# locuslab/mpc.pytorch

Measured on NVIDIA H100. Metric: LQR solves/sec, higher is better.
Workload: dtype f32

## Files before the change

### include/mpcb200.h

```cpp
#ifndef MPCB200_H_
#define MPCB200_H_

#include <stddef.h>
#include <stdint.h>

#ifdef __cplusplus
extern "C" {
#endif

#define MPCB200_VERSION 2

enum {
  MPCB200_OK = 0,
  MPCB200_ERR_NULL_POINTER = 1,
  MPCB200_ERR_BAD_DIMS = 2,
  MPCB200_ERR_UNSUPPORTED_DIMS = 3,
  MPCB200_ERR_SMEM = 4,
  MPCB200_ERR_LAUNCH = 5,
  MPCB200_ERR_NO_DEVICE = 6,
  MPCB200_ERR_NO_GRAPH_COND = 7
};

typedef struct mpcb200_dims {
  int32_t B;
// ... 105 lines not shown
} mpcb200_ilqr_opts;

size_t mpcb200_ilqr_workspace_bytes(const mpcb200_dims* dims, const mpcb200_ilqr_opts* opts, int32_t elem_size);
int mpcb200_ilqr_f32(const mpcb200_dims* dims, const mpcb200_params* params, const mpcb200_ilqr_opts* opts,
                     const float* C, const float* c, const float* F, const float* f,
                     const float* x_init, const float* u_init,
                     const float* u_lower, const float* u_upper, const uint8_t* u_zero_I,
                     float* best_x, float* best_u, float* best_costs, float* best_full_du_norm,
                     int32_t* info, void* workspace, size_t workspace_bytes, void* stream);
int mpcb200_ilqr_f64(const mpcb200_dims* dims, const mpcb200_params* params, const mpcb200_ilqr_opts* opts,
                     const double* C, const double* c, const double* F, const double* f,
                     const double* x_init, const double* u_init,
                     const double* u_lower, const double* u_upper, const uint8_t* u_zero_I,
                     double* best_x, double* best_u, double* best_costs, double* best_full_du_norm,
                     int32_t* info, void* workspace, size_t workspace_bytes, void* stream);

int mpcb200_supported(int32_t n_state, int32_t n_ctrl);

int mpcb200_supported_list(int32_t* out, int32_t cap);

uint64_t mpcb200_launch_count(void);

size_t mpcb200_step_smem_bytes(const mpcb200_dims* dims, int32_t elem_size);

int mpcb200_step_prefers_workspace(const mpcb200_dims* dims, int32_t elem_size);

#define MPCB200_PLAN_GENERIC 1u
#define MPCB200_PLAN_PAIR 2u
#define MPCB200_PLAN_GAINS_SMEM 4u
#define MPCB200_PLAN_KREDUCE 8u
#define MPCB200_PLAN_LARGE 16u
int32_t mpcb200_last_step_plan(void);

int mpcb200_version(void);
const char* mpcb200_strerror(int code);

#ifdef __cplusplus
}
#endif
#endif
```

### mpc/pytorch_b200/_lib.py

```python
import contextlib
import ctypes
import functools
import os

import torch

_HERE = os.path.dirname(os.path.abspath(__file__))
LIB_PATH = os.environ.get("MPCB200_LIB", os.path.join(_HERE, "libmpcb200.so"))


class Dims(ctypes.Structure):
    _fields_ = [(k, ctypes.c_int32) for k in (
        "B", "T", "n", "m", "F_T", "has_f", "bounds_kind", "has_zero_mask",
        "has_delta_u", "max_ls_iter", "pnqp_max_iter", "do_rollout", "dynamics_kind", "reserved0")] + \
        [(k, ctypes.c_int64) for k in ("C_tstride", "c_tstride", "F_tstride", "f_tstride")]



class Params(ctypes.Structure):
    _fields_ = [(k, ctypes.c_double) for k in ("u_lo", "u_hi", "delta_u", "ls_decay")] + [("dyn", ctypes.c_double * 8)]


class IlqrOpts(ctypes.Structure):
    _fields_ = [(k, ctypes.c_int32) for k in ("lqr_iter", "not_improved_lim", "m_ref", "reserved0")] + \
        [(k, ctypes.c_double) for k in ("eps", "best_cost_eps")]


class MpcB200Error(RuntimeError):
    pass


ERR_NO_GRAPH_COND = 7


_lib = None

EXPORTED_SYMBOLS = (
    "mpcb200_lqr_step_f32", "mpcb200_lqr_step_f64", "mpcb200_lqr_grad_f32", "mpcb200_lqr_grad_f64",
    "mpcb200_rollout_f32", "mpcb200_rollout_f64", "mpcb200_pnqp_f32", "mpcb200_pnqp_f64", "mpcb200_pnqp_max_n",
    "mpcb200_lqr_adjoint_f32", "mpcb200_lqr_adjoint_f64", "mpcb200_adjoint_workspace_bytes",
    "mpcb200_dyn_rollout_f32", "mpcb200_dyn_rollout_f64", "mpcb200_dyn_linearize_f32", "mpcb200_dyn_linearize_f64",
    "mpcb200_supported", "mpcb200_supported_list", "mpcb200_launch_count",
    "mpcb200_step_smem_bytes", "mpcb200_step_prefers_workspace", "mpcb200_last_step_plan", "mpcb200_version",
    "mpcb200_strerror", "mpcb200_step_large_fits", "mpcb200_ilqr_f32", "mpcb200_ilqr_f64",
    "mpcb200_ilqr_workspace_bytes",
)

PLAN_GENERIC, PLAN_PAIR, PLAN_GAINS_SMEM, PLAN_KREDUCE, PLAN_LARGE = 1, 2, 4, 8, 16


def lib():
    global _lib
    if _lib is not None:
        return _lib
    if not os.path.exists(LIB_PATH):
        raise MpcB200Error(
            f"{LIB_PATH} is not built. Run `python -c 'import __graft_entry__ as g; g.build()'` "
            "(or `make -C mpc/pytorch_b200/csrc`). There is no CPU fallback.")
    L = ctypes.CDLL(LIB_PATH)
    vp = ctypes.c_void_p
    step_args = [ctypes.POINTER(Dims), ctypes.POINTER(Params)] + [vp] * 22
    for name in ("mpcb200_lqr_step_f32", "mpcb200_lqr_step_f64"):
        fn = getattr(L, name)
        fn.argtypes = step_args
        fn.restype = ctypes.c_int
    grad_args = [ctypes.POINTER(Dims)] + [vp] * 15
    for name in ("mpcb200_lqr_grad_f32", "mpcb200_lqr_grad_f64"):
        fn = getattr(L, name)
        fn.argtypes = grad_args
        fn.restype = ctypes.c_int
    for name in ("mpcb200_rollout_f32", "mpcb200_rollout_f64"):
        fn = getattr(L, name)
        fn.argtypes = [ctypes.POINTER(Dims)] + [vp] * 6
        fn.restype = ctypes.c_int
    for name in ("mpcb200_pnqp_f32", "mpcb200_pnqp_f64"):
        fn = getattr(L, name)
        fn.argtypes = [ctypes.c_int32, ctypes.c_int32] + [vp] * 5 + [ctypes.c_int32] + [vp] * 6
        fn.restype = ctypes.c_int
# ... 4 lines not shown
        fn.argtypes = [ctypes.POINTER(Dims), ctypes.POINTER(Params)] + [vp] * 15 + [ctypes.c_size_t, vp]
        fn.restype = ctypes.c_int
    L.mpcb200_adjoint_workspace_bytes.argtypes = [ctypes.POINTER(Dims), ctypes.c_int32]
    L.mpcb200_adjoint_workspace_bytes.restype = ctypes.c_size_t
    for name in ("mpcb200_dyn_rollout_f32", "mpcb200_dyn_rollout_f64"):
        fn = getattr(L, name)
        fn.argtypes = [ctypes.c_int32, ctypes.POINTER(ctypes.c_double), ctypes.c_int32, ctypes.c_int32] + [vp] * 4
        fn.restype = ctypes.c_int
    for name in ("mpcb200_dyn_linearize_f32", "mpcb200_dyn_linearize_f64"):
        fn = getattr(L, name)
        fn.argtypes = [ctypes.c_int32, ctypes.POINTER(ctypes.c_double), ctypes.c_int32, ctypes.c_int32] + [vp] * 5
        fn.restype = ctypes.c_int
    for name in ("mpcb200_ilqr_f32", "mpcb200_ilqr_f64"):
        fn = getattr(L, name)
        fn.argtypes = [ctypes.POINTER(Dims), ctypes.POINTER(Params), ctypes.POINTER(IlqrOpts)] + [vp] * 15 + \
            [ctypes.c_size_t, vp]
        fn.restype = ctypes.c_int
    L.mpcb200_ilqr_workspace_bytes.argtypes = [ctypes.POINTER(Dims), ctypes.POINTER(IlqrOpts), ctypes.c_int32]
    L.mpcb200_ilqr_workspace_bytes.restype = ctypes.c_size_t
    L.mpcb200_supported.argtypes = [ctypes.c_int32, ctypes.c_int32]
    L.mpcb200_supported.restype = ctypes.c_int
    L.mpcb200_supported_list.argtypes = [ctypes.POINTER(ctypes.c_int32), ctypes.c_int32]
    L.mpcb200_supported_list.restype = ctypes.c_int
    L.mpcb200_launch_count.argtypes = []
    L.mpcb200_launch_count.restype = ctypes.c_uint64
    L.mpcb200_step_smem_bytes.argtypes = [ctypes.POINTER(Dims), ctypes.c_int32]
    L.mpcb200_step_smem_bytes.restype = ctypes.c_size_t
    L.mpcb200_step_prefers_workspace.argtypes = [ctypes.POINTER(Dims), ctypes.c_int32]
    L.mpcb200_step_prefers_workspace.restype = ctypes.c_int
    L.mpcb200_step_large_fits.argtypes = [ctypes.POINTER(Dims), ctypes.c_int32]
    L.mpcb200_step_large_fits.restype = ctypes.c_int
    L.mpcb200_last_step_plan.argtypes = []
    L.mpcb200_last_step_plan.restype = ctypes.c_int32
    L.mpcb200_version.argtypes = []
    L.mpcb200_version.restype = ctypes.c_int
    L.mpcb200_strerror.argtypes = [ctypes.c_int]
    L.mpcb200_strerror.restype = ctypes.c_char_p
    _lib = L
    return L


_DTYPE_SUFFIX = {torch.float32: "_f32", torch.float64: "_f64"}


@functools.cache
def entry(name, dtype):
    suffix = _DTYPE_SUFFIX.get(dtype)
    if suffix is None:
        raise MpcB200Error(f"unsupported dtype {dtype}")
    return getattr(lib(), name + suffix)


def check(rc, what):
    if rc != 0:
        raise MpcB200Error(f"{what} failed: [{rc}] {lib().mpcb200_strerror(rc).decode()}")


def supported_pairs():
    L = lib()
    n = L.mpcb200_supported_list(None, 0)
    buf = (ctypes.c_int32 * (2 * n))()
    L.mpcb200_supported_list(buf, n)
    return [(buf[2 * i], buf[2 * i + 1]) for i in range(n)]


def launch_count():
    return int(lib().mpcb200_launch_count())


def last_step_plan():
    return int(lib().mpcb200_last_step_plan())


def ptr(t):
    if t is None:
        return None
    if not t.is_cuda:
        raise MpcB200Error("mpc.pytorch_b200 runs on CUDA tensors only (no CPU fallback)")
    if not t.is_contiguous():
        raise MpcB200Error("internal error: non-contiguous tensor reached the C ABI")
    return ctypes.c_void_p(t.data_ptr())


def ptr_view(t):
    if t is None:
        return None
    if not t.is_cuda:
        raise MpcB200Error("mpc.pytorch_b200 runs on CUDA tensors only (no CPU fallback)")
    return ctypes.c_void_p(t.data_ptr())


def stream_handle(device):
    return ctypes.c_void_p(torch.cuda.current_stream(device).cuda_stream)


def _on_device(dev):
    if dev.index is None or dev.index == torch.cuda.current_device():
        return contextlib.nullcontext()
    return torch.cuda.device(dev)
```

### mpc/pytorch_b200/csrc/api.cu

```cuda
#include <atomic>
#include <cstdlib>
#include <cstring>

#include "../../../include/mpcb200.h"
#include "ilqr.cuh"
#include "lqr_grad.cuh"
#include "lqr_large.cuh"
#include "lqr_rollout.cuh"
#include "lqr_step.cuh"
#include "pnqp.cuh"

namespace mpcb200 {
#define MPCB200_INST(n, m)                                                  \
  int step_f32__##n##_##m(const StepArgs&, int, cudaStream_t);              \
  int step_f64__##n##_##m(const StepArgs&, int, cudaStream_t);              \
  int grad_f32__##n##_##m(const GradArgs&, cudaStream_t);                   \
  int grad_f64__##n##_##m(const GradArgs&, cudaStream_t);                   \
  int pws_f32__##n##_##m(int, int);                                         \
  int pws_f64__##n##_##m(int, int);                                         \
  int roll_f32__##n##_##m(const RolloutArgs&, cudaStream_t);                \
  int roll_f64__##n##_##m(const RolloutArgs&, cudaStream_t);                \
  size_t smem_f32__##n##_##m(int);                                          \
  size_t smem_f64__##n##_##m(int);
#include "instances.def"
// ... 7 lines not shown
  int (*grad64)(const GradArgs&, cudaStream_t);
  size_t (*smem32)(int);
  size_t (*smem64)(int);
  int (*roll32)(const RolloutArgs&, cudaStream_t);
  int (*roll64)(const RolloutArgs&, cudaStream_t);
  int (*pws32)(int, int);
  int (*pws64)(int, int);
};
static const Entry kTable[] = {
#define MPCB200_INST(n, m)                                                                  \
  {n, m, step_f32__##n##_##m, step_f64__##n##_##m, grad_f32__##n##_##m, grad_f64__##n##_##m, \
   smem_f32__##n##_##m, smem_f64__##n##_##m, roll_f32__##n##_##m, roll_f64__##n##_##m,   \
   pws_f32__##n##_##m, pws_f64__##n##_##m},
#include "instances.def"
#undef MPCB200_INST
};
static const int kTableLen = (int)(sizeof(kTable) / sizeof(kTable[0]));

static const Entry* find(int n, int m) {
  for (int i = 0; i < kTableLen; ++i)
    if (kTable[i].n == n && kTable[i].m == m) return &kTable[i];
  return nullptr;
}

static bool large_forced() {
  const char* k = std::getenv("MPCB200_KERNEL");
  return k != nullptr && std::atoi(k) == 3;
}
static bool runs_large(int n, int m) { return find(n, m) == nullptr || large_forced(); }
static constexpr int kOptinAssumed = 227 * 1024;

static std::atomic<uint64_t> g_launches{0};
static thread_local int t_step_plan = 0;

void record_step_plan(int plan) { t_step_plan = plan; }

int max_smem_optin() {
  static std::atomic<int> cache[64];
  int dev = 0;
  if (cudaGetDevice(&dev) != cudaSuccess) return -1;
  if (dev < 0 || dev >= 64) return -1;
  if (cache[dev].load(std::memory_order_acquire) == 0) {
    int v = 0, major = 0;
    if (cudaDeviceGetAttribute(&v, cudaDevAttrMaxSharedMemoryPerBlockOptin, dev) != cudaSuccess) return -1;
    if (cudaDeviceGetAttribute(&major, cudaDevAttrComputeCapabilityMajor, dev) != cudaSuccess) return -1;
    if (major != 9) return -1;
    cache[dev].store(v, std::memory_order_release);
  }
  return cache[dev].load(std::memory_order_acquire);
}

struct TimeStrides { long long C, c, F, f; };
static TimeStrides time_strides(const mpcb200_dims* d) {
  auto ts = [](long long given, long long dense) { return given == 0 ? dense : (given < 0 ? 0 : given); };
  const long long B = d->B, n = d->n, p = d->n + d->m;
  return {ts(d->C_tstride, B * p * p), ts(d->c_tstride, B * p), ts(d->F_tstride, B * n * p), ts(d->f_tstride, B * n)};
}

static bool aligned16(const void* p) { return (reinterpret_cast<uintptr_t>(p) & 15u) == 0; }

static int check_dims(const mpcb200_dims* d) {
  if (d == nullptr) return MPCB200_ERR_NULL_POINTER;
  if (d->B <= 0 || d->T <= 0 || d->n <= 0 || d->m <= 0) return MPCB200_ERR_BAD_DIMS;
  if (d->F_T != d->T - 1 && d->F_T != d->T) return MPCB200_ERR_BAD_DIMS;
  return MPCB200_OK;
}

static int check_bounds(const mpcb200_dims* d, const void* lo, const void* hi) {
// ... 67 lines not shown
  const size_t sz = sizeof(R);
  bool ok = aligned16(C) && aligned16(c) && aligned16(cur_x) && aligned16(cur_u) &&
            (F == nullptr || aligned16(F)) && (!d->has_f || aligned16(f)) &&
            (d->bounds_kind != 2 || (aligned16(u_lower) && aligned16(u_upper)));
  ok = ok && (x_init == nullptr || aligned16(x_init));
  ok = ok && ((size_t)d->B * d->m * sz) % 16 == 0 && ((size_t)d->B * d->n * sz) % 16 == 0;
  a.bulk_ok = ok ? 1 : 0;
  const TimeStrides ts = time_strides(d);
  a.C_ts = ts.C; a.c_ts = ts.c; a.F_ts = ts.F; a.f_ts = ts.f;
  ok = ok && (a.C_ts * sz) % 16 == 0 && (a.c_ts * sz) % 16 == 0 && (a.F_ts * sz) % 16 == 0 && (a.f_ts * sz) % 16 == 0;
  a.bulk_ok = ok ? 1 : 0;
  a.dyn_kind = d->dynamics_kind;
  if (a.dyn_kind != DYN_LINEAR) {
    if (!known_shape_ok(d)) return MPCB200_ERR_BAD_DIMS;
    for (int i = 0; i < 8; ++i) a.dp.p[i] = p->dyn[i];
  }
  if (large) {
    if (adj != nullptr) return MPCB200_ERR_UNSUPPORTED_DIMS;
    if (Ks == nullptr) return MPCB200_ERR_SMEM;
    const int n = d->n, m = d->m, p = n + m;
    auto spans = [&](const void* base, long long ts, long long span) {
      return base != nullptr && aligned16(base) && (ts * (long long)sz) % 16 == 0 && (span * (long long)sz) % 16 == 0;
    };
    unsigned bulk = 0u;
    if (spans(C, a.C_ts, (long long)p * p)) bulk |= LB_C;
    if (spans(F, a.F_ts, (long long)n * p)) bulk |= LB_F;
    if (spans(c, a.c_ts, p)) bulk |= LB_c;
    if (d->has_f && spans(f, a.f_ts, n)) bulk |= LB_f;
    if (spans(cur_x, (long long)d->B * n, n)) bulk |= LB_x;
    if (spans(cur_u, (long long)d->B * m, m)) bulk |= LB_u;
    if (d->bounds_kind == 2 && spans(u_lower, (long long)d->B * m, m) && spans(u_upper, (long long)d->B * m, m))
      bulk |= LB_BOX;
    t_step_plan = 0;
    rc = large_step_launch<R>(a, n, m, bulk, smem, (cudaStream_t)stream);
    if (rc == 0) g_launches.fetch_add(1);
    return rc;
  }
  if (const char* k = std::getenv("MPCB200_KERNEL")) a.impl = std::atoi(k);
  if (adj != nullptr) {
    if (!adj->ok || !a.bulk_ok || a.impl == 1) return MPCB200_ERR_UNSUPPORTED_DIMS;
    a.impl = 2;
    a.adj = 1; a.adj_has_df = adj->has_df; a.adj_c = adj->c; a.adj_x = adj->x; a.adj_u = adj->u;
    a.adj_dC = adj->dC; a.adj_dc = adj->dc; a.adj_dF = adj->dF; a.adj_df = adj->df; a.adj_dx_init = adj->dx_init;
    a.adj_c_ts = adj->c_ts;
  }
  t_step_plan = 0;
  rc =(sizeof(R) == 4 ? e->step32 : e->step64)(a, smem, (cudaStream_t)stream);
  if (rc == 0) g_launches.fetch_add(1);
  return rc;
}

template <typename R>
static int grad_impl(const mpcb200_dims* d, const R* C, const R* c, const R* F, const R* new_x,
                     const R* new_u, const R* dx, const R* du, const R* dl_dx, R* dx_init, R* dC, R* dc,
                     R* dF, R* df, void* workspace, void* stream) {
  int rc = check_dims(d);
  if (rc) return rc;
  if (C == nullptr || c == nullptr || new_x == nullptr || new_u == nullptr || dx == nullptr ||
      du == nullptr || dl_dx == nullptr || dx_init == nullptr || dC == nullptr || dc == nullptr)
    return MPCB200_ERR_NULL_POINTER;
  if (d->F_T > 0 && (F == nullptr || dF == nullptr)) return MPCB200_ERR_NULL_POINTER;
  const Entry* e = find(d->n, d->m);
  const bool large = runs_large(d->n, d->m);
  if (max_smem_optin() <= 0) return MPCB200_ERR_NO_DEVICE;
  GradArgs a;
  std::memset(&a, 0, sizeof(a));
  a.B = d->B; a.T = d->T; a.F_T = d->F_T; a.has_df = df != nullptr;
  a.C = C; a.c = c; a.F = F; a.new_x = new_x; a.new_u = new_u; a.dx = dx; a.du = du; a.dl_dx = dl_dx;
  a.dx_init = dx_init; a.dC = dC; a.dc = dc; a.dF = dF; a.df = df; a.workspace = workspace;
  const TimeStrides ts = time_strides(d);
  a.C_ts = ts.C; a.c_ts = ts.c; a.F_ts = ts.F;
  rc = large ? large_grad_launch<R>(a, d->n, d->m, (cudaStream_t)stream)
             : (sizeof(R) == 4 ? e->grad32 : e->grad64)(a, (cudaStream_t)stream);
  if (rc == 0) g_launches.fetch_add(workspace != nullptr ? 2 : 1);
  return rc;
}
struct AdjLayout {
  size_t negr, zeros, dx, du, costate, scal, mask, maskf, Ks, ks, total;
  bool gains;
// ... 482 lines not shown
int mpcb200_supported_list(int32_t* out, int32_t cap) {
  for (int i = 0; i < kTableLen && i < cap; ++i) {
    out[2 * i] = kTable[i].n;
    out[2 * i + 1] = kTable[i].m;
  }
  return kTableLen;
}

uint64_t mpcb200_launch_count(void) { return g_launches.load(); }

size_t mpcb200_step_smem_bytes(const mpcb200_dims* dims, int32_t elem_size) {
  if (dims == nullptr) return 0;
  const Entry* e = find(dims->n, dims->m);
  if (e == nullptr) return 0;
  return elem_size == 8 ? e->smem64(dims->T) : e->smem32(dims->T);
}

int mpcb200_step_prefers_workspace(const mpcb200_dims* dims, int32_t elem_size) {
  if (dims == nullptr) return 0;
  if (runs_large(dims->n, dims->m)) return 1;
  const Entry* e = find(dims->n, dims->m);
  int ms = max_smem_optin();
  if (ms <= 0) ms = kOptinAssumed;
  return elem_size == 8 ? e->pws64(dims->T, ms) : e->pws32(dims->T, ms);
}

int mpcb200_step_large_fits(const mpcb200_dims* dims, int32_t elem_size) {
  if (dims == nullptr || (elem_size != 4 && elem_size != 8)) return 0;
  return large_step_fits(dims->n, dims->m, elem_size, kOptinAssumed) ? 1 : 0;
}

int32_t mpcb200_last_step_plan(void) { return t_step_plan; }

int mpcb200_version(void) { return MPCB200_VERSION; }

const char* mpcb200_strerror(int code) {
  switch (code) {
    case MPCB200_OK: return "ok";
    case MPCB200_ERR_NULL_POINTER: return "a required pointer is NULL";
    case MPCB200_ERR_BAD_DIMS: return "bad dimensions or option combination";
    case MPCB200_ERR_UNSUPPORTED_DIMS: return "no kernel instance compiled for this (n_state, n_ctrl)";
    case MPCB200_ERR_SMEM: return "problem does not fit shared memory (pass Ks/ks buffers for long horizons)";
    case MPCB200_ERR_LAUNCH: return "CUDA launch failed";
    case MPCB200_ERR_NO_DEVICE: return "no usable sm_90 device";
    case MPCB200_ERR_NO_GRAPH_COND: return "conditional CUDA graph nodes are unavailable (driver older than 12.3)";
    default: return "unknown error";
  }
}
}
```

### mpc/pytorch_b200/csrc/lqr_step.cuh

```cuda
#pragma once
#include "../../../include/mpcb200.h"
#include "common.cuh"
#include "dynamics.cuh"

namespace mpcb200 {

struct StepArgs {
  int B, T, F_T;
  int has_f, bounds_kind, has_mask, has_delta, max_ls, pnqp_iters, do_rollout;
  double u_lo, u_hi, delta_u, ls_decay;
  const void *C, *c, *F, *f, *x_init, *cur_x, *cur_u, *u_lower, *u_upper;
  const unsigned char* zero_mask;
  void *new_x, *new_u, *costs, *full_du_norm, *alphas, *du_first;
  int* qp_iters;
  unsigned char* free_mask;
  int* status;
  void *Ks, *ks;
  int bulk_ok;
  int k_in_smem;
  int impl;
  long long C_ts, c_ts, F_ts, f_ts;
  int adj, adj_has_df;
  const void *adj_c, *adj_x, *adj_u;
  void *adj_dC, *adj_dc, *adj_dF, *adj_df, *adj_dx_init;
  long long adj_c_ts;
  int dyn_kind;
  DynParams dp;
};

void record_step_plan(int plan);

template <typename R, int N, int M>
struct StepCfg {
  static constexpr int P = N + M;
  static constexpr int EA = 16 / (int)sizeof(R);
  static_assert(P <= 32, "one problem must fit a warp");
  static constexpr bool STATE_LANES = N == 8 && M == 2 && sizeof(R) == 4;
  static constexpr int LP = STATE_LANES ? N : P;
  static constexpr int CPL = (P + LP - 1) / LP;
  static constexpr int PPW = 32 / LP;
  static constexpr bool x_slot(int sl) { return sl * LP < N; }
  static constexpr bool span_ok(int nw) {
    return (nw * PPW * M * (int)sizeof(R)) % 16 == 0 && (nw * PPW * N * (int)sizeof(R)) % 16 == 0;
  }
  static constexpr int NW = STATE_LANES ? 2 : span_ok(1) ? 1 : span_ok(2) ? 2 : 4;
  static constexpr int W = NW * PPW;
  static_assert(span_ok(NW), "CTA problem count must keep spans 16-byte aligned");
  static constexpr int THREADS = (NW + 1) * 32;
  static constexpr int MIN_CTAS = STATE_LANES ? 32 / W : 0;
  static constexpr int S = 3;
  static constexpr int VS = round_up(N, 4);
  static constexpr int CS = P * P, FS = N * P;
  static constexpr int OFF_C = 0;
  static constexpr int OFF_F = OFF_C + W * CS;
  static constexpr int OFF_c = OFF_F + W * FS;
  static constexpr int OFF_f = OFF_c + W * P;
  static constexpr int OFF_x = OFF_f + W * N;
  static constexpr int OFF_u = OFF_x + W * N;
  static constexpr int OFF_lo = OFF_u + W * M;
  static constexpr int OFF_hi = OFF_lo + W * M;
  static constexpr int OFF_END = OFF_hi + W * M;
  static constexpr int STAGE_BYTES = round_up(OFF_END * (int)sizeof(R) + round_up(W * M, 16), 128);
  static constexpr int SC_V = 0;
  static constexpr int SC_v = SC_V + N * VS;
  static constexpr int SC_K = SC_v + VS;
  static constexpr int KT = M * VS + round_up(M, 4);
  static constexpr int SC_Q = SC_K + KT;
  static constexpr int SC_R = SC_Q + M * VS;
  static constexpr int SC_RAW = SC_R + round_up(P, 4);
  static constexpr int SCR = (SC_RAW % 32 == 0 || SC_RAW % 32 == 16) ? SC_RAW + 4 : SC_RAW;
  static constexpr bool KREDUCE = CPL == 1 && PPW == 1 && (N & (N - 1)) == 0;
  static constexpr int GAIN_SMEM_LIMIT = 6144;
  static bool prefers_workspace(int T, int max_smem_optin) {
    return smem_bytes(T, true) > (size_t)max_smem_optin ||
           (KREDUCE && (size_t)T * KT * sizeof(R) > (size_t)GAIN_SMEM_LIMIT);
  }
  static constexpr int HDR_BYTES = 256;
  static size_t smem_bytes(int T, bool k_in_smem) {
    size_t b = HDR_BYTES + (size_t)S * STAGE_BYTES + (size_t)W * SCR * sizeof(R);
    if (k_in_smem) b += (size_t)W * T * KT * sizeof(R);
    return b;
  }
};

template <typename R, int M>
MPCB_DEV void pnqp_lane(const R (&H)[M][M], const R (&q)[M], const R (&lo)[M], const R (&hi)[M],
                        bool warm, R (&x)[M], Ldl<R, M>& fac, unsigned& fmask, int& iters,
                        bool& conv, bool& badpiv, int max_iter) {
  const R GAMMA = R(0.1);
  auto obj = [&](const R(&z)[M]) {
    R s = R(0);
#pragma unroll
    for (int a = 0; a < M; ++a) {
      R hz = R(0);
#pragma unroll
      for (int b = 0; b < M; ++b) hz += H[a][b] * z[b];
      s += z[a] * (R(0.5) * hz + q[a]);
    }
    return s;
  };
  badpiv = false;
  if (!warm) {
    fac.factor(H);
    badpiv = fac.bad;
    R t[M];
    fac.solve(q, t);
#pragma unroll
    for (int a = 0; a < M; ++a) x[a] = -t[a];
  }
#pragma unroll
  for (int a = 0; a < M; ++a) {
    x[a] = x[a] < lo[a] ? lo[a] : x[a];
    x[a] = x[a] > hi[a] ? hi[a] : x[a];
  }

// ... 153 lines not shown
      const R l2 = ubar - du, h2 = ubar + du;
      lo = l2 < lo ? lo : l2;
      hi = h2 > hi ? hi : h2;
    }
    u = u < lo ? lo : u;
    u = u > hi ? hi : u;
  }
  return u;
}

template <typename R>
MPCB_DEV bool line_search_update(int pass, R cost, R oldcost, R du2, R decay, R& fdn, R& alpha) {
  if (pass == 0) fdn = sqrt(du2);
  const bool worse = cost > oldcost;
  if (worse) alpha *= decay;
  return worse;
}

MPCB_DEV void write_step_status(const StepArgs& a, int b, unsigned status) {
  if (a.status != nullptr) a.status[b] = (int)status;
}

template <typename R>
MPCB_DEV void write_step_result(const StepArgs& a, int b, R alpha, R cost, R fdn, unsigned status) {
  ((R*)a.costs)[b] = cost;
  ((R*)a.full_du_norm)[b] = fdn;
  ((R*)a.alphas)[b] = alpha;
  if (!(cost - cost == R(0))) status |= MPCB200_ST_NONFINITE;
  write_step_status(a, b, status);
}

template <typename R, int N, int M>
MPCB_DEV void step_producer(const StepArgs& a, unsigned char* stage_base, uint64_t* full,
                            uint64_t* empty, volatile int* votes, int b0, int cnt, int lane) {
  using K = StepCfg<R, N, M>;
  constexpr int P = K::P;
  constexpr uint32_t SZ = sizeof(R);
  const R* gC = (const R*)a.C;
  const R* gc = (const R*)a.c;
  const R* gF = (const R*)a.F;
  const R* gf = (const R*)a.f;
  const R* gx = (const R*)a.cur_x;
  const R* gu = (const R*)a.cur_u;
  const R* glo = (const R*)a.u_lower;
  const R* ghi = (const R*)a.u_upper;
  const bool tail_ok = (cnt == K::W) || (((cnt * M * SZ) % 16 == 0) && ((cnt * N * SZ) % 16 == 0));
  const bool bulk = a.bulk_ok && tail_ok;
  const int T = a.T;
  int s = 0;
  uint32_t ph = 0;
  const uint64_t last_use = l2_evict_first_policy();
  auto g2s = [&](void* dst, const void* src, uint32_t bytes, uint64_t* bar, bool fwd) {
    if (fwd) bulk_g2s(dst, src, bytes, bar, last_use);
    else bulk_g2s(dst, src, bytes, bar);
  };

  auto issue = [&](int t, bool fwd) {
    mbar_wait(&empty[s], ph ^ 1u);
    R* st = (R*)(stage_base + (size_t)s * K::STAGE_BYTES);
    const size_t tb = (size_t)t * a.B + b0;
    const size_t tC = (size_t)t * a.C_ts + (size_t)b0 * P * P, tF = (size_t)t * a.F_ts + (size_t)b0 * N * P;
    const size_t tc = (size_t)t * a.c_ts + (size_t)b0 * P, tf_ = (size_t)t * a.f_ts + (size_t)b0 * N;
    const bool needF = t < T - 1;
    const bool needf = fwd && needF && a.has_f;
    if (a.has_mask) {
      unsigned char* mk = (unsigned char*)(st + K::OFF_END);
      for (int i = lane; i < cnt * M; i += 32) mk[i] = a.zero_mask[tb * M + i];
    }
    if (bulk) {
      __syncwarp();
      if (lane == 0) {
        uint32_t bytes = (uint32_t)cnt * (P * P + P + N + M) * SZ;
        if (needF) bytes += (uint32_t)cnt * N * P * SZ;
        if (needf) bytes += (uint32_t)cnt * N * SZ;
        if (a.bounds_kind == 2) bytes += 2u * cnt * M * SZ;
        mbar_arrive_expect_tx(&full[s], bytes);
        if constexpr (K::CS == P * P) {
          g2s(st + K::OFF_C, gC + tC, (uint32_t)cnt * P * P * SZ, &full[s], fwd);
        } else {
          for (int q = 0; q < cnt; ++q)
            g2s(st + K::OFF_C + q * K::CS, gC + tC + (size_t)q * P * P, (uint32_t)P * P * SZ, &full[s], fwd);
        }
        if (needF) {
          if constexpr (K::FS == N * P) {
            g2s(st + K::OFF_F, gF + tF, (uint32_t)cnt * N * P * SZ, &full[s], fwd);
          } else {
            for (int q = 0; q < cnt; ++q)
              g2s(st + K::OFF_F + q * K::FS, gF + tF + (size_t)q * N * P, (uint32_t)N * P * SZ, &full[s], fwd);
          }
        }
        g2s(st + K::OFF_c, gc + tc, (uint32_t)cnt * P * SZ, &full[s], fwd);
        if (needf) g2s(st + K::OFF_f, gf + tf_, (uint32_t)cnt * N * SZ, &full[s], fwd);
        g2s(st + K::OFF_x, gx + tb * N, (uint32_t)cnt * N * SZ, &full[s], fwd);
        g2s(st + K::OFF_u, gu + tb * M, (uint32_t)cnt * M * SZ, &full[s], fwd);
        if (a.bounds_kind == 2) {
          g2s(st + K::OFF_lo, glo + tb * M, (uint32_t)cnt * M * SZ, &full[s], fwd);
          g2s(st + K::OFF_hi, ghi + tb * M, (uint32_t)cnt * M * SZ, &full[s], fwd);
        }
      }
    } else {
      auto cp = [&](R* dst, const R* src, int nelem) {
        for (int i = lane; i < nelem; i += 32) dst[i] = __ldg(src + i);
      };
      for (int q = 0; q < cnt; ++q) cp(st + K::OFF_C + q * K::CS, gC + tC + (size_t)q * P * P, P * P);
      if (needF)
        for (int q = 0; q < cnt; ++q) cp(st + K::OFF_F + q * K::FS, gF + tF + (size_t)q * N * P, N * P);
      cp(st + K::OFF_c, gc + tc, cnt * P);
      if (needf) cp(st + K::OFF_f, gf + tf_, cnt * N);
      cp(st + K::OFF_x, gx + tb * N, cnt * N);
      cp(st + K::OFF_u, gu + tb * M, cnt * M);
      if (a.bounds_kind == 2) {
        cp(st + K::OFF_lo, glo + tb * M, cnt * M);
        cp(st + K::OFF_hi, ghi + tb * M, cnt * M);
      }
      __syncwarp();
      if (lane == 0) mbar_arrive(&full[s]);
    }
    if (++s == K::S) { s = 0; ph ^= 1u; }
  };

  for (int t = T - 1; t >= 0; --t) issue(t, false);
  if (a.do_rollout) {
    for (int pass = 0;; ++pass) {
      for (int t = 0; t < T; ++t) issue(t, true);
      named_bar_sync(1, K::THREADS);
      const int cont = votes[pass & 31];
      if (!cont || pass + 1 >= a.max_ls) break;
    }
  }
}



template <typename R, int N, int M, int MODE>
MPCB_DEV void step_consumer(const StepArgs& a, unsigned char* stage_base, uint64_t* full,
                            uint64_t* empty, volatile int* votes, R* scratch_all, R* kstore_all,
                            int b0, int warp, int lane) {
  using K = StepCfg<R, N, M>;
  constexpr int P = K::P, LP = K::LP, PPW = K::PPW, CPL = K::CPL, VS = K::VS, EA = K::EA, KT = K::KT;
  constexpr unsigned FULLM = (1u << M) - 1u;
  constexpr bool BOX = MODE == MODE_BOX;
  constexpr int A_N = align_elems<R>(N), A_M = align_elems<R>(M);
  constexpr int A_ROW = (P % 2 == 0) ? 2 : 1;
  constexpr int A_2P = align_elems<R>(2 * P), A_NP = align_elems<R>(K::FS);
  const int T = a.T, B = a.B;
  const bool writer_lane = lane < PPW * LP;
  const int pi = writer_lane ? lane / LP : PPW - 1;
  const int base = pi * LP;
  const int j = writer_lane ? lane - base : LP - 1;
  const int pw = warp * PPW + pi;
  const int b = b0 + pw;
  const bool valid = b < B;
  const bool wr = writer_lane && valid;

  int cc[CPL], ua[CPL], fr[CPL];
  bool isx[CPL], wsl[CPL];
#pragma unroll
  for (int sl = 0; sl < CPL; ++sl) {
    const int col = j + sl * LP;
    wsl[sl] = writer_lane && col < P;
    cc[sl] = col < P ? col : P - 1;
    isx[sl] = K::x_slot(sl) && cc[sl] < N;
    ua[sl] = isx[sl] ? 0 : cc[sl] - N;
    fr[sl] = isx[sl] ? cc[sl] : N - 1;
  }

  const int oC = K::OFF_C + pw * K::CS, oF = K::OFF_F + pw * K::FS;
  const int oc = K::OFF_c + pw * P, of_ = K::OFF_f + pw * N, ox = K::OFF_x + pw * N, ou = K::OFF_u + pw * M;
  const int olo = K::OFF_lo + pw * M, ohi = K::OFF_hi + pw * M;

  R* scr = scratch_all + (size_t)pw * K::SCR;
  R* Vs = scr + K::SC_V;
  R* vs = scr + K::SC_v;
  R* Qx = scr + K::SC_Q;
  R* red = scr + K::SC_R;
  R* kst = a.k_in_smem ? kstore_all + (size_t)pw * T * KT : scr + K::SC_K;
  R* gKs = (R*)a.Ks;
  R* gks = (R*)a.ks;

  const R s_lo = (R)a.u_lo, s_hi = (R)a.u_hi, s_du = (R)a.delta_u;
  const R decay = (R)a.ls_decay;
  const bool has_mask = MODE == MODE_MASK || (BOX && a.has_mask);

  int stg = 0;
  uint32_t ph = 0;
  unsigned status = 0u;
  R oldcost_part = R(0), oldcost_slot[CPL] = {};
  R kprev[M];
#pragma unroll
  for (int q = 0; q < M; ++q) kprev[q] = R(0);

  for (int t = T - 1; t >= 0; --t) {
    mbar_wait(&full[stg], ph);
    const R* st = (const R*)(stage_base + (size_t)stg * K::STAGE_BYTES);
    const unsigned char* mk = (const unsigned char*)(st + K::OFF_END) + pw * M;

    Vec<R, P> tb;
    {
      Vec<R, N> tx;
      Vec<R, M> tu;
      tx.template load<A_N>(st + ox);
      tu.template load<A_M>(st + ou);
#pragma unroll
      for (int i = 0; i < N; ++i) tb.set(i, tx.get(i));
#pragma unroll
      for (int q = 0; q < M; ++q) tb.set(N + q, tu.get(q));
      if constexpr (P & 1) tb.p[Vec<R, P>::NP - 1].y = R(0);
    }
    Vec<R, P> Qc[CPL];
    R qj[CPL];
#pragma unroll
    for (int sl = 0; sl < CPL; ++sl) {
      Qc[sl].gather(st + oC + cc[sl], P);
      Vec<R, P> Crow;
      Crow.template load<A_ROW>(st + oC + cc[sl] * P);
      const R Ct = Crow.dot(tb);
      const R cj = st[oc + cc[sl]];
      const R tbj = st[(isx[sl] ? ox : ou - N) + cc[sl]];
      if constexpr (CPL == 1) {
        if (wsl[sl]) oldcost_part += tbj * (R(0.5) * Ct + cj);
      } else {
        if (wsl[sl]) oldcost_slot[sl] += tbj * (R(0.5) * Ct + cj);
      }
      qj[sl] = Ct + cj;
    }
    if (t < T - 1) {
      Vec<R, N> Fcol[CPL], Wc[CPL];
// ... 148 lines not shown
        R sacc = Qc[sl].get(N + p1);
#pragma unroll
        for (int p2 = 0; p2 < M; ++p2) sacc += Quu[p1][p2] * Kc[sl][p2];
        G[sl][p1] = sacc;
      }
#pragma unroll
      for (int i = 0; i < N; ++i) Vn[sl].set(i, Qc[sl].get(i));
      if constexpr (N & 1) Vn[sl].p[Vec<R, N>::NP - 1].y = R(0);
      vn[sl] = qj[sl];
    }
#pragma unroll
    for (int q = 0; q < M; ++q) {
      Vec<R, N> Qrow, Krow;
      Qrow.template load<EA>(Qx + q * VS);
      Krow.template load<EA>(Kt + q * VS);
      R sacc = qu[q];
#pragma unroll
      for (int p2 = 0; p2 < M; ++p2) sacc += Quu[q][p2] * kk[p2];
#pragma unroll
      for (int sl = 0; sl < CPL; ++sl) {
        Vn[sl].axpy(Qrow, Kc[sl][q]);
        Vn[sl].axpy(Krow, G[sl][q]);
        vn[sl] += Qx[q * VS + fr[sl]] * kk[q] + Kc[sl][q] * sacc;
      }
    }
#pragma unroll
    for (int sl = 0; sl < CPL; ++sl) {
      if (wsl[sl] && isx[sl]) {
        Vn[sl].template store<EA>(Vs + cc[sl] * VS);
        vs[cc[sl]] = vn[sl];
      }
    }
    __syncwarp();
    if (lane == 0) mbar_arrive(&empty[stg]);
    if (++stg == K::S) { stg = 0; ph ^= 1u; }
  }

  if constexpr (CPL == 1) {
    if (writer_lane) red[j] = oldcost_part;
  } else {
#pragma unroll
    for (int sl = 0; sl < CPL; ++sl)
      if (wsl[sl]) red[cc[sl]] = oldcost_slot[sl];
  }
  __syncwarp();
  R oldcost = R(0);
#pragma unroll
  for (int i = 0; i < P; ++i) oldcost += red[i];
  __syncwarp();

  if (!a.do_rollout) {
    if (wr && j == 0) write_step_status(a, b, status);
    return;
  }

  const R* gx0 = (const R*)a.x_init;
  R* gnx = (R*)a.new_x;
  R* gnu = (R*)a.new_u;
  R* gdu1 = (R*)a.du_first;
  R alpha = R(1), fdn = R(0), cost = R(0);
  bool worse = false;
  for (int pass = 0;; ++pass) {
    Vec<R, N> xr;
#pragma unroll
    for (int i = 0; i < N; ++i) xr.set(i, valid ? gx0[(size_t)b * N + i] : R(0));
    if constexpr (N & 1) xr.p[Vec<R, N>::NP - 1].y = R(0);
    R xown[CPL];
#pragma unroll
    for (int sl = 0; sl < CPL; ++sl) xown[sl] = valid ? gx0[(size_t)b * N + fr[sl]] : R(0);
    R cpart = R(0), cpart_slot[CPL] = {}, dun2 = R(0);
    R kcol[M], kff[M];
#pragma unroll
    for (int q = 0; q < M; ++q) {
      kcol[q] = R(0);
      kff[q] = R(0);
    }
    if constexpr (K::KREDUCE) {
      if (!a.k_in_smem) {
        const size_t kb = (size_t)(valid ? b : 0) * M;
#pragma unroll
        for (int q = 0; q < M; ++q) {
          kcol[q] = __ldcg(gKs + (kb + q) * N + fr[0]);
          kff[q] = __ldcg(gks + kb + q);
        }
      }
    }
    size_t orow = (size_t)b;
    for (int t = 0; t < T; ++t, orow += (size_t)B) {
      mbar_wait(&full[stg], ph);
      const R* st = (const R*)(stage_base + (size_t)stg * K::STAGE_BYTES);
      const unsigned char* mk = (const unsigned char*)(st + K::OFF_END) + pw * M;

      Vec<R, N> xb, dxv;
      Vec<R, M> ubar;
      xb.template load<A_N>(st + ox);
      ubar.template load<A_M>(st + ou);
#pragma unroll
      for (int k2 = 0; k2 < Vec<R, N>::NP; ++k2) dxv.p[k2] = fma2(xb.p[k2], P2<R>{R(-1), R(-1)}, xr.p[k2]);
      R u[M];
      if (a.k_in_smem) {
        const R* Kt = kst + (size_t)t * KT;
#pragma unroll
        for (int q = 0; q < M; ++q) {
          Vec<R, N> Krow;
          Krow.template load<EA>(Kt + q * VS);
          u[q] = (Krow.dot(dxv) + ubar.get(q)) + alpha * Kt[M * VS + q];
        }
      } else if constexpr (K::KREDUCE) {
        const R dxi = xown[0] - st[ox + fr[0]];
        R part[M];
#pragma unroll
        for (int q = 0; q < M; ++q) part[q] = isx[0] ? kcol[q] * dxi : R(0);
#pragma unroll
        for (int off = N / 2; off >= 1; off >>= 1) {
#pragma unroll
          for (int q = 0; q < M; ++q) part[q] += __shfl_xor_sync(0xffffffffu, part[q], off);
        }
#pragma unroll
        for (int q = 0; q < M; ++q) u[q] = (shfl(part[q], base) + ubar.get(q)) + alpha * kff[q];
        if (t + 1 < T) {
          const size_t kb = ((size_t)(t + 1) * B + (valid ? b : 0)) * M;
#pragma unroll
          for (int q = 0; q < M; ++q) {
// ... 64 lines not shown
          }
        }
        xn[sl] = R(0);
        if (K::x_slot(sl) && t < T - 1) {
          bool known = false;
          if constexpr (M == 1 && (N == DynDims<DYN_CARTPOLE>::N || N == DynDims<DYN_PENDULUM>::N)) {
            if (a.dyn_kind != DYN_LINEAR) {
              known = true;
              R sv[N], ov[N];
#pragma unroll
              for (int i = 0; i < N; ++i) sv[i] = tau.get(i);
              dyn_step<R, N == DynDims<DYN_CARTPOLE>::N ? DYN_CARTPOLE : DYN_PENDULUM, R>(a.dp, sv, tau.get(N), ov);
              xn[sl] = ov[0];
#pragma unroll
              for (int i = 1; i < N; ++i)
                if (fr[sl] == i) xn[sl] = ov[i];
            }
          }
          if (!known) {
            Vec<R, P> Frow;
            Frow.template load<A_ROW>(st + oF + fr[sl] * P);
            xn[sl] = Frow.dot(tau);
            if (a.has_f) xn[sl] += st[of_ + fr[sl]];
          }
        }
      }
      if (t < T - 1) {
#pragma unroll
        for (int i = 0; i < N; ++i) xr.set(i, shfl(xn[i / LP], base + i % LP));
#pragma unroll
        for (int sl = 0; sl < CPL; ++sl) xown[sl] = xn[sl];
      }
      __syncwarp();
      if (lane == 0) mbar_arrive(&empty[stg]);
      if (++stg == K::S) { stg = 0; ph ^= 1u; }
    }
    if constexpr (CPL == 1) {
      if (writer_lane) red[j] = cpart;
    } else {
#pragma unroll
      for (int sl = 0; sl < CPL; ++sl)
        if (wsl[sl]) red[cc[sl]] = cpart_slot[sl];
    }
    __syncwarp();
    cost = R(0);
#pragma unroll
    for (int i = 0; i < P; ++i) cost += red[i];
    __syncwarp();
    worse = line_search_update<R>(pass, cost, oldcost, dun2, decay, fdn, alpha);
    const bool more = pass + 1 < a.max_ls;
    if (wr && j == 0 && worse && more) votes[pass & 31] = 1;
    if (warp == 0 && lane == 0) votes[(pass + 16) & 31] = 0;
    named_bar_sync(1, K::THREADS);
    const int cont = votes[pass & 31];
    if (!cont || !more) break;
  }
  if (worse) alpha /= decay;
  if (wr && j == 0) write_step_result<R>(a, b, alpha, cost, fdn, status);
}

template <typename R, int N, int M, int MODE>
__global__ void __launch_bounds__(StepCfg<R, N, M>::THREADS, StepCfg<R, N, M>::MIN_CTAS)
lqr_step_kernel(const StepArgs a) {
  using K = StepCfg<R, N, M>;
  extern __shared__ __align__(128) unsigned char smem_raw[];
  uint64_t* full = reinterpret_cast<uint64_t*>(smem_raw);
  uint64_t* empty = full + K::S;
  volatile int* votes = reinterpret_cast<volatile int*>(smem_raw + 128);
  unsigned char* stage_base = smem_raw + K::HDR_BYTES;
  R* scratch = reinterpret_cast<R*>(stage_base + (size_t)K::S * K::STAGE_BYTES);
  R* kstore = scratch + (size_t)K::W * K::SCR;

  const int tid = threadIdx.x, warp = tid >> 5, lane = tid & 31;
  const int b0 = blockIdx.x * K::W;
  const int cnt = min(K::W, a.B - b0);
  if (tid == 0) {
#pragma unroll
    for (int s = 0; s < K::S; ++s) {
      mbar_init(&full[s], 1);
      mbar_init(&empty[s], K::NW);
    }
    mbar_fence_init();
  }
  if (tid < 32) votes[tid] = 0;
  __syncthreads();
  if (warp == K::NW) {
    step_producer<R, N, M>(a, stage_base, full, empty, votes, b0, cnt, lane);
  } else {
    step_consumer<R, N, M, MODE>(a, stage_base, full, empty, votes, scratch, kstore, b0, warp, lane);
  }
}

template <typename R, int N, int M, int MODE>
int launch_step_mode(const StepArgs& args, int max_smem_optin, cudaStream_t stream) {
  using K = StepCfg<R, N, M>;
  StepArgs a = args;
  size_t smem;
  int rc = plan_gain_store(a, K::prefers_workspace(a.T, max_smem_optin), max_smem_optin,
                           [&](bool k_in_smem) { return K::smem_bytes(a.T, k_in_smem); }, smem);
  if (rc == MPCB200_OK) rc = allow_smem_optin<lqr_step_kernel<R, N, M, MODE>>(max_smem_optin);
  if (rc != MPCB200_OK) return rc;
  const int grid = (a.B + K::W - 1) / K::W;
  lqr_step_kernel<R, N, M, MODE><<<grid, K::THREADS, smem, stream>>>(a);
  if (cudaGetLastError() != cudaSuccess) return MPCB200_ERR_LAUNCH;
  record_step_plan((int)(MPCB200_PLAN_GENERIC | (a.k_in_smem ? MPCB200_PLAN_GAINS_SMEM : 0u) |
                         (K::KREDUCE && !a.k_in_smem && a.do_rollout ? MPCB200_PLAN_KREDUCE : 0u)));
  return MPCB200_OK;
}

template <typename R, int N, int M>
int launch_step(const StepArgs& a, int max_smem_optin, cudaStream_t stream) {
  if (a.bounds_kind != 0) return launch_step_mode<R, N, M, MODE_BOX>(a, max_smem_optin, stream);
  if (a.has_mask) return launch_step_mode<R, N, M, MODE_MASK>(a, max_smem_optin, stream);
  return launch_step_mode<R, N, M, MODE_PLAIN>(a, max_smem_optin, stream);
}

template <typename R, int N, int M>
int step_prefers_workspace(int T, int max_smem_optin) {
  return StepCfg<R, N, M>::prefers_workspace(T, max_smem_optin) ? 1 : 0;
}

template <typename R, int N, int M>
size_t step_smem_query(int T) {
  return StepCfg<R, N, M>::smem_bytes(T, true);
}

}
```

Before: 88.88 million.

## Pin trailing timestep tiles in spare shared memory and reuse ring tiles across sweeps

Spare shared memory left over at the current occupancy now holds a number of timestep tiles, taken from the end of the horizon. These tiles are loaded once during the backward sweep and reused by the forward rollout without being fetched again. The ring-buffer stage mapping is also rearranged so the last few ring tiles loaded in the backward sweep stay resident for the first rollout pass. The aim is to cut global and L2 traffic from re-streaming C, F, x and u on every line-search pass. In exchange, per-stage phase tracking becomes more complex, occupancy queries add host overhead, and the changed stage indexing carries correctness risk.

```diff
diff --git a/include/mpcb200.h b/include/mpcb200.h
--- a/include/mpcb200.h
+++ b/include/mpcb200.h
@@ -161,6 +161,10 @@
 #define MPCB200_PLAN_LARGE 16u
 int32_t mpcb200_last_step_plan(void);
 
+#define MPCB200_TILES_PINNED(v) ((v) & 0xffff)
+#define MPCB200_TILES_RING(v) (((v) >> 16) & 0xff)
+int32_t mpcb200_last_step_tiles(void);
+
 int mpcb200_version(void);
 const char* mpcb200_strerror(int code);
 
diff --git a/mpc/pytorch_b200/_lib.py b/mpc/pytorch_b200/_lib.py
--- a/mpc/pytorch_b200/_lib.py
+++ b/mpc/pytorch_b200/_lib.py
@@ -43,7 +43,7 @@
     "mpcb200_supported", "mpcb200_supported_list", "mpcb200_launch_count",
     "mpcb200_step_smem_bytes", "mpcb200_step_prefers_workspace", "mpcb200_last_step_plan", "mpcb200_version",
     "mpcb200_strerror", "mpcb200_step_large_fits", "mpcb200_ilqr_f32", "mpcb200_ilqr_f64",
-    "mpcb200_ilqr_workspace_bytes",
+    "mpcb200_ilqr_workspace_bytes", "mpcb200_last_step_tiles",
 )
 
 PLAN_GENERIC, PLAN_PAIR, PLAN_GAINS_SMEM, PLAN_KREDUCE, PLAN_LARGE = 1, 2, 4, 8, 16
@@ -114,6 +114,8 @@
     L.mpcb200_step_large_fits.restype = ctypes.c_int
     L.mpcb200_last_step_plan.argtypes = []
     L.mpcb200_last_step_plan.restype = ctypes.c_int32
+    L.mpcb200_last_step_tiles.argtypes = []
+    L.mpcb200_last_step_tiles.restype = ctypes.c_int32
     L.mpcb200_version.argtypes = []
     L.mpcb200_version.restype = ctypes.c_int
     L.mpcb200_strerror.argtypes = [ctypes.c_int]
@@ -154,6 +156,11 @@
     return int(lib().mpcb200_last_step_plan())
 
 
+def last_step_tiles():
+    v = int(lib().mpcb200_last_step_tiles())
+    return v & 0xffff, (v >> 16) & 0xff
+
+
 def ptr(t):
     if t is None:
         return None
diff --git a/mpc/pytorch_b200/csrc/api.cu b/mpc/pytorch_b200/csrc/api.cu
--- a/mpc/pytorch_b200/csrc/api.cu
+++ b/mpc/pytorch_b200/csrc/api.cu
@@ -63,8 +63,10 @@
 
 static std::atomic<uint64_t> g_launches{0};
 static thread_local int t_step_plan = 0;
+static thread_local int t_step_tiles = 0;
 
 void record_step_plan(int plan) { t_step_plan = plan; }
+void record_step_tiles(int pinned, int ring) { t_step_tiles = pinned | (ring << 16); }
 
 int max_smem_optin() {
   static std::atomic<int> cache[64];
@@ -198,6 +200,7 @@
     if (d->bounds_kind == 2 && spans(u_lower, (long long)d->B * m, m) && spans(u_upper, (long long)d->B * m, m))
       bulk |= LB_BOX;
     t_step_plan = 0;
+    t_step_tiles = 0;
     rc = large_step_launch<R>(a, n, m, bulk, smem, (cudaStream_t)stream);
     if (rc == 0) g_launches.fetch_add(1);
     return rc;
@@ -211,6 +214,7 @@
     a.adj_c_ts = adj->c_ts;
   }
   t_step_plan = 0;
+  t_step_tiles = 0;
   rc =(sizeof(R) == 4 ? e->step32 : e->step64)(a, smem, (cudaStream_t)stream);
   if (rc == 0) g_launches.fetch_add(1);
   return rc;
@@ -759,6 +763,8 @@
 
 int32_t mpcb200_last_step_plan(void) { return t_step_plan; }
 
+int32_t mpcb200_last_step_tiles(void) { return t_step_tiles; }
+
 int mpcb200_version(void) { return MPCB200_VERSION; }
 
 const char* mpcb200_strerror(int code) {
diff --git a/mpc/pytorch_b200/csrc/lqr_step.cuh b/mpc/pytorch_b200/csrc/lqr_step.cuh
--- a/mpc/pytorch_b200/csrc/lqr_step.cuh
+++ b/mpc/pytorch_b200/csrc/lqr_step.cuh
@@ -1,4 +1,7 @@
 #pragma once
+#include <map>
+#include <mutex>
+#include <utility>
 #include "../../../include/mpcb200.h"
 #include "common.cuh"
 #include "dynamics.cuh"
@@ -19,6 +22,7 @@
   int bulk_ok;
   int k_in_smem;
   int impl;
+  int pins;
   long long C_ts, c_ts, F_ts, f_ts;
   int adj, adj_has_df;
   const void *adj_c, *adj_x, *adj_u;
@@ -29,6 +33,7 @@
 };
 
 void record_step_plan(int plan);
+void record_step_tiles(int pinned, int ring);
 
 template <typename R, int N, int M>
 struct StepCfg {
@@ -81,6 +86,15 @@
     if (k_in_smem) b += (size_t)W * T * KT * sizeof(R);
     return b;
   }
+  __host__ __device__ static constexpr int pin_offset(int T, bool k_in_smem) {
+    return round_up(HDR_BYTES + S * STAGE_BYTES + W * SCR * (int)sizeof(R) + (k_in_smem ? W * T * KT * (int)sizeof(R) : 0),
+                    128);
+  }
+  static size_t smem_bytes(int T, bool k_in_smem, int pins) {
+    return pins == 0 ? smem_bytes(T, k_in_smem) : (size_t)pin_offset(T, k_in_smem) + (size_t)pins * (STAGE_BYTES + 8);
+  }
+  __host__ __device__ static constexpr int sweep_stage(int ring_tiles, int t) { return (ring_tiles - 1 - t) % S; }
+  __host__ __device__ static constexpr int rollout_stage(int ring_tiles, int t) { return (ring_tiles - 1 - t % S) % S; }
 };
 
 template <typename R, int M>
@@ -300,7 +314,8 @@
 
 template <typename R, int N, int M>
 MPCB_DEV void step_producer(const StepArgs& a, unsigned char* stage_base, uint64_t* full,
-                            uint64_t* empty, volatile int* votes, int b0, int cnt, int lane) {
+                            uint64_t* empty, unsigned char* pin_base, uint64_t* pin_full, volatile int* votes,
+                            int b0, int cnt, int lane) {
   using K = StepCfg<R, N, M>;
   constexpr int P = K::P;
   constexpr uint32_t SZ = sizeof(R);
@@ -314,8 +329,8 @@
   const R* ghi = (const R*)a.u_upper;
   const bool tail_ok = (cnt == K::W) || (((cnt * M * SZ) % 16 == 0) && ((cnt * N * SZ) % 16 == 0));
   const bool bulk = a.bulk_ok && tail_ok;
-  const int T = a.T;
-  int s = 0;
+  const int T = a.T, TR = T - a.pins;
+  const int r = a.do_rollout ? min(K::S, TR) : 0;
   uint32_t ph = 0;
   const uint64_t last_use = l2_evict_first_policy();
   auto g2s = [&](void* dst, const void* src, uint32_t bytes, uint64_t* bar, bool fwd) {
@@ -323,9 +338,7 @@
     else bulk_g2s(dst, src, bytes, bar);
   };
 
-  auto issue = [&](int t, bool fwd) {
-    mbar_wait(&empty[s], ph ^ 1u);
-    R* st = (R*)(stage_base + (size_t)s * K::STAGE_BYTES);
+  auto issue = [&](int t, bool fwd, R* st, uint64_t* bar) {
     const size_t tb = (size_t)t * a.B + b0;
     const size_t tC = (size_t)t * a.C_ts + (size_t)b0 * P * P, tF = (size_t)t * a.F_ts + (size_t)b0 * N * P;
     const size_t tc = (size_t)t * a.c_ts + (size_t)b0 * P, tf_ = (size_t)t * a.f_ts + (size_t)b0 * N;
@@ -342,28 +355,28 @@
         if (needF) bytes += (uint32_t)cnt * N * P * SZ;
         if (needf) bytes += (uint32_t)cnt * N * SZ;
         if (a.bounds_kind == 2) bytes += 2u * cnt * M * SZ;
-        mbar_arrive_expect_tx(&full[s], bytes);
+        mbar_arrive_expect_tx(bar, bytes);
         if constexpr (K::CS == P * P) {
-          g2s(st + K::OFF_C, gC + tC, (uint32_t)cnt * P * P * SZ, &full[s], fwd);
+          g2s(st + K::OFF_C, gC + tC, (uint32_t)cnt * P * P * SZ, bar, fwd);
         } else {
           for (int q = 0; q < cnt; ++q)
-            g2s(st + K::OFF_C + q * K::CS, gC + tC + (size_t)q * P * P, (uint32_t)P * P * SZ, &full[s], fwd);
+            g2s(st + K::OFF_C + q * K::CS, gC + tC + (size_t)q * P * P, (uint32_t)P * P * SZ, bar, fwd);
         }
         if (needF) {
           if constexpr (K::FS == N * P) {
-            g2s(st + K::OFF_F, gF + tF, (uint32_t)cnt * N * P * SZ, &full[s], fwd);
+            g2s(st + K::OFF_F, gF + tF, (uint32_t)cnt * N * P * SZ, bar, fwd);
           } else {
             for (int q = 0; q < cnt; ++q)
-              g2s(st + K::OFF_F + q * K::FS, gF + tF + (size_t)q * N * P, (uint32_t)N * P * SZ, &full[s], fwd);
+              g2s(st + K::OFF_F + q * K::FS, gF + tF + (size_t)q * N * P, (uint32_t)N * P * SZ, bar, fwd);
           }
         }
-        g2s(st + K::OFF_c, gc + tc, (uint32_t)cnt * P * SZ, &full[s], fwd);
-        if (needf) g2s(st + K::OFF_f, gf + tf_, (uint32_t)cnt * N * SZ, &full[s], fwd);
-        g2s(st + K::OFF_x, gx + tb * N, (uint32_t)cnt * N * SZ, &full[s], fwd);
-        g2s(st + K::OFF_u, gu + tb * M, (uint32_t)cnt * M * SZ, &full[s], fwd);
+        g2s(st + K::OFF_c, gc + tc, (uint32_t)cnt * P * SZ, bar, fwd);
+        if (needf) g2s(st + K::OFF_f, gf + tf_, (uint32_t)cnt * N * SZ, bar, fwd);
+        g2s(st + K::OFF_x, gx + tb * N, (uint32_t)cnt * N * SZ, bar, fwd);
+        g2s(st + K::OFF_u, gu + tb * M, (uint32_t)cnt * M * SZ, bar, fwd);
         if (a.bounds_kind == 2) {
-          g2s(st + K::OFF_lo, glo + tb * M, (uint32_t)cnt * M * SZ, &full[s], fwd);
-          g2s(st + K::OFF_hi, ghi + tb * M, (uint32_t)cnt * M * SZ, &full[s], fwd);
+          g2s(st + K::OFF_lo, glo + tb * M, (uint32_t)cnt * M * SZ, bar, fwd);
+          g2s(st + K::OFF_hi, ghi + tb * M, (uint32_t)cnt * M * SZ, bar, fwd);
         }
       }
     } else {
@@ -382,15 +395,21 @@
         cp(st + K::OFF_hi, ghi + tb * M, cnt * M);
       }
       __syncwarp();
-      if (lane == 0) mbar_arrive(&full[s]);
-    }
-    if (++s == K::S) { s = 0; ph ^= 1u; }
+      if (lane == 0) mbar_arrive(bar);
+    }
   };
-
-  for (int t = T - 1; t >= 0; --t) issue(t, false);
+  auto issue_ring = [&](int t, bool fwd, int s) {
+    mbar_wait(&empty[s], ((ph >> s) & 1u) ^ 1u);
+    ph ^= 1u << s;
+    issue(t, fwd, (R*)(stage_base + (size_t)s * K::STAGE_BYTES), &full[s]);
+  };
+
+  for (int t = T - 1; t >= TR; --t)
+    issue(t, true, (R*)(pin_base + (size_t)(T - 1 - t) * K::STAGE_BYTES), &pin_full[T - 1 - t]);
+  for (int t = TR - 1; t >= 0; --t) issue_ring(t, t < r, K::sweep_stage(TR, t));
   if (a.do_rollout) {
     for (int pass = 0;; ++pass) {
-      for (int t = 0; t < T; ++t) issue(t, true);
+      for (int t = pass == 0 ? r : 0; t < TR; ++t) issue_ring(t, true, K::rollout_stage(TR, t));
       named_bar_sync(1, K::THREADS);
       const int cont = votes[pass & 31];
       if (!cont || pass + 1 >= a.max_ls) break;
@@ -402,8 +421,8 @@
 
 template <typename R, int N, int M, int MODE>
 MPCB_DEV void step_consumer(const StepArgs& a, unsigned char* stage_base, uint64_t* full,
-                            uint64_t* empty, volatile int* votes, R* scratch_all, R* kstore_all,
-                            int b0, int warp, int lane) {
+                            uint64_t* empty, unsigned char* pin_base, uint64_t* pin_full, volatile int* votes,
+                            R* scratch_all, R* kstore_all, int b0, int warp, int lane) {
   using K = StepCfg<R, N, M>;
   constexpr int P = K::P, LP = K::LP, PPW = K::PPW, CPL = K::CPL, VS = K::VS, EA = K::EA, KT = K::KT;
   constexpr unsigned FULLM = (1u << M) - 1u;
@@ -450,7 +469,8 @@
   const R decay = (R)a.ls_decay;
   const bool has_mask = MODE == MODE_MASK || (BOX && a.has_mask);
 
-  int stg = 0;
+  const int TR = T - a.pins;
+  const int r = a.do_rollout ? min(K::S, TR) : 0;
   uint32_t ph = 0;
   unsigned status = 0u;
   R oldcost_part = R(0), oldcost_slot[CPL] = {};
@@ -459,8 +479,16 @@
   for (int q = 0; q < M; ++q) kprev[q] = R(0);
 
   for (int t = T - 1; t >= 0; --t) {
-    mbar_wait(&full[stg], ph);
-    const R* st = (const R*)(stage_base + (size_t)stg * K::STAGE_BYTES);
+    const int stg = t < TR ? K::sweep_stage(TR, t) : -1;
+    const R* st;
+    if (stg < 0) {
+      mbar_wait(&pin_full[T - 1 - t], 0u);
+      st = (const R*)(pin_base + (size_t)(T - 1 - t) * K::STAGE_BYTES);
+    } else {
+      mbar_wait(&full[stg], (ph >> stg) & 1u);
+      ph ^= 1u << stg;
+      st = (const R*)(stage_base + (size_t)stg * K::STAGE_BYTES);
+    }
     const unsigned char* mk = (const unsigned char*)(st + K::OFF_END) + pw * M;
 
     Vec<R, P> tb;
@@ -675,8 +703,7 @@
       }
     }
     __syncwarp();
-    if (lane == 0) mbar_arrive(&empty[stg]);
-    if (++stg == K::S) { stg = 0; ph ^= 1u; }
+    if (lane == 0 && stg >= 0 && t >= r) mbar_arrive(&empty[stg]);
   }
 
   if constexpr (CPL == 1) {
@@ -730,8 +757,17 @@
     }
     size_t orow = (size_t)b;
     for (int t = 0; t < T; ++t, orow += (size_t)B) {
-      mbar_wait(&full[stg], ph);
-      const R* st = (const R*)(stage_base + (size_t)stg * K::STAGE_BYTES);
+      const int stg = t < TR ? K::rollout_stage(TR, t) : -1;
+      const R* st;
+      if (stg < 0) {
+        st = (const R*)(pin_base + (size_t)(T - 1 - t) * K::STAGE_BYTES);
+      } else {
+        if (pass > 0 || t >= r) {
+          mbar_wait(&full[stg], (ph >> stg) & 1u);
+          ph ^= 1u << stg;
+        }
+        st = (const R*)(stage_base + (size_t)stg * K::STAGE_BYTES);
+      }
       const unsigned char* mk = (const unsigned char*)(st + K::OFF_END) + pw * M;
 
       Vec<R, N> xb, dxv;
@@ -862,8 +898,7 @@
         for (int sl = 0; sl < CPL; ++sl) xown[sl] = xn[sl];
       }
       __syncwarp();
-      if (lane == 0) mbar_arrive(&empty[stg]);
-      if (++stg == K::S) { stg = 0; ph ^= 1u; }
+      if (lane == 0 && stg >= 0) mbar_arrive(&empty[stg]);
     }
     if constexpr (CPL == 1) {
       if (writer_lane) red[j] = cpart;
@@ -900,6 +935,8 @@
   unsigned char* stage_base = smem_raw + K::HDR_BYTES;
   R* scratch = reinterpret_cast<R*>(stage_base + (size_t)K::S * K::STAGE_BYTES);
   R* kstore = scratch + (size_t)K::W * K::SCR;
+  unsigned char* pin_base = smem_raw + K::pin_offset(a.T, a.k_in_smem);
+  uint64_t* pin_full = reinterpret_cast<uint64_t*>(pin_base + (size_t)a.pins * K::STAGE_BYTES);
 
   const int tid = threadIdx.x, warp = tid >> 5, lane = tid & 31;
   const int b0 = blockIdx.x * K::W;
@@ -910,15 +947,65 @@
       mbar_init(&full[s], 1);
       mbar_init(&empty[s], K::NW);
     }
+    for (int i = 0; i < a.pins; ++i) mbar_init(&pin_full[i], 1);
     mbar_fence_init();
   }
   if (tid < 32) votes[tid] = 0;
   __syncthreads();
   if (warp == K::NW) {
-    step_producer<R, N, M>(a, stage_base, full, empty, votes, b0, cnt, lane);
+    step_producer<R, N, M>(a, stage_base, full, empty, pin_base, pin_full, votes, b0, cnt, lane);
   } else {
-    step_consumer<R, N, M, MODE>(a, stage_base, full, empty, votes, scratch, kstore, b0, warp, lane);
-  }
+    step_consumer<R, N, M, MODE>(a, stage_base, full, empty, pin_base, pin_full, votes, scratch, kstore, b0, warp,
+                                 lane);
+  }
+}
+
+template <auto Kern>
+int resident_ctas(int threads, size_t smem) {
+  static std::mutex mu;
+  static std::map<std::pair<int, size_t>, int> cache;
+  int dev = 0;
+  if (cudaGetDevice(&dev) != cudaSuccess) return 0;
+  std::lock_guard<std::mutex> lock(mu);
+  const auto key = std::make_pair(dev, smem);
+  auto it = cache.find(key);
+  if (it != cache.end()) return it->second;
+  int n = 0;
+  if (cudaOccupancyMaxActiveBlocksPerMultiprocessor(&n, Kern, threads, smem) != cudaSuccess) {
+    (void)cudaGetLastError();
+    n = 0;
+  }
+  cache.emplace(key, n);
+  return n;
+}
+
+inline int device_sm_count() {
+  static std::atomic<int> cache[64];
+  int dev = 0;
+  if (cudaGetDevice(&dev) != cudaSuccess || dev < 0 || dev >= 64) return 0;
+  if (cache[dev].load(std::memory_order_acquire) == 0) {
+    int v = 0;
+    if (cudaDeviceGetAttribute(&v, cudaDevAttrMultiProcessorCount, dev) != cudaSuccess) return 0;
+    cache[dev].store(v, std::memory_order_release);
+  }
+  return cache[dev].load(std::memory_order_acquire);
+}
+
+template <typename R, int N, int M, int MODE>
+int plan_pins(const StepArgs& a, int grid, size_t smem, int max_smem_optin) {
+  using K = StepCfg<R, N, M>;
+  constexpr auto kern = lqr_step_kernel<R, N, M, MODE>;
+  if (!a.do_rollout) return 0;
+  const int occ = resident_ctas<kern>(K::THREADS, smem), sms = device_sm_count();
+  if (occ <= 0 || sms <= 0) return 0;
+  const int need = min(occ, (grid + sms - 1) / sms);
+  int pins = 0;
+  while (pins < a.T) {
+    const size_t s = K::smem_bytes(a.T, a.k_in_smem, pins + 1);
+    if (s > (size_t)max_smem_optin || resident_ctas<kern>(K::THREADS, s) < need) break;
+    ++pins;
+  }
+  return pins;
 }
 
 template <typename R, int N, int M, int MODE>
@@ -931,10 +1018,13 @@
   if (rc == MPCB200_OK) rc = allow_smem_optin<lqr_step_kernel<R, N, M, MODE>>(max_smem_optin);
   if (rc != MPCB200_OK) return rc;
   const int grid = (a.B + K::W - 1) / K::W;
+  a.pins = plan_pins<R, N, M, MODE>(a, grid, smem, max_smem_optin);
+  smem = K::smem_bytes(a.T, a.k_in_smem, a.pins);
   lqr_step_kernel<R, N, M, MODE><<<grid, K::THREADS, smem, stream>>>(a);
   if (cudaGetLastError() != cudaSuccess) return MPCB200_ERR_LAUNCH;
   record_step_plan((int)(MPCB200_PLAN_GENERIC | (a.k_in_smem ? MPCB200_PLAN_GAINS_SMEM : 0u) |
                          (K::KREDUCE && !a.k_in_smem && a.do_rollout ? MPCB200_PLAN_KREDUCE : 0u)));
+  record_step_tiles(a.pins, a.do_rollout ? min(K::S, a.T - a.pins) : 0);
   return MPCB200_OK;
 }
 
```

Result: no change. 89.48 million, median of 6 (+0.7%).
